# VCISwang/STCD

Hardware: AMD Instinct MI355X
Metric: image-pairs/sec (256x256 bf16 SiamUnet_diff train) (higher is better)
Workload: dtype bf16; 1 GPU; SiamUnet_diff(3,2) 256x256 full training step (fwd + cross_entropy + bwd + AdamW), 16 pairs/GPU, synthetic LEVIR-CD-shaped pairs resident in HBM; global_batch=16, image=256, parallelism=dp1

## Files before the change

### include/stcd_hip.h

```cpp
#ifndef STCD_HIP_H
#define STCD_HIP_H

#include <stdint.h>

#ifdef __cplusplus
extern "C" {
#endif

#define STCD_ABI_VERSION 2

#define STCD_ARCH_DIFF 0
#define STCD_ARCH_CONC 1
#define STCD_ARCH_SUB 2
#define STCD_ARCH_SNUNET 3
#define STCD_ARCH_SEGCD 4
#define STCD_ARCH_SEGCD_R18 5
#define STCD_ARCH_SEGCD_R34 6
#define STCD_ARCH_SEGCD_R101 7
#define STCD_ARCH_SEGCD_R152 8
#define STCD_ARCH_FCEF 9
#define STCD_ARCH_XCONC 10
#define STCD_ARCH_SNUNET_CONC 11
#define STCD_ARCH_SNUNET_CONC_DS 12
#define STCD_ARCH_UNETSEG 16
// ... 213 lines not shown
    int32_t bw_ldy;
    int32_t blocks, tiles_per_group, blocks_per_group, bn_rep;
    int32_t tile_m;
} stcd_conv_fused;
int stcd_op_conv_fused(const stcd_conv_geom* g, stcd_conv_fused* f, const void* in, const float* w, const float* bias, void* out,
                       void* scratch, int64_t scratch_bytes, void* hip_stream);
int stcd_op_wgrad(int dtype, int impl, const stcd_conv_geom* g, const void* in, const void* dout, float* dw,
                  void* scratch, int64_t scratch_bytes, void* hip_stream);
int64_t stcd_op_scratch_bytes(const stcd_conv_geom* g);

typedef struct stcd_map_geom {
    int32_t n, h, w, c, groups;
} stcd_map_geom;
int64_t stcd_op_ew_scratch_bytes(const stcd_map_geom* g);
int stcd_op_bn_act(int dtype, const stcd_map_geom* g, const void* y, int ldy, const float* gamma, const float* beta,
                   float* running_mean, float* running_var, const float* mask, int relu, int training, void* a, int lda,
                   void* pool, int ldp, float* stat, void* scratch, int64_t scratch_bytes, void* hip_stream);
int stcd_op_bn_act_pair(int dtype, const stcd_map_geom* g, const void* y, int ldy, const float* gamma, const float* beta,
                        float* running_mean, float* running_var, const float* mask, int fuse_mode, void* a, int lda, void* pool,
                        int ldp, void* fused, int ldf, float* stat, void* scratch, int64_t scratch_bytes, void* hip_stream);
int stcd_op_bn_act_bwd(int dtype, const stcd_map_geom* g, const void* da, int ldda, const void* y, int ldy, const float* stat,
                       const float* mask, int relu, void* dy, int lddy, float* dgamma, float* dbeta, void* scratch,
                       int64_t scratch_bytes, void* hip_stream);
int stcd_op_maxpool(int dtype, const stcd_map_geom* g, const void* a, int lda, void* pool, int ldp, void* hip_stream);
int stcd_op_maxpool_bwd(int dtype, const stcd_map_geom* g, const void* a, int lda, const void* dpool, int ldp, void* da, int ldda,
                        int accumulate, void* hip_stream);
int stcd_op_maxpool3(int dtype, const stcd_map_geom* g, const void* a, int lda, void* pool, int ldp, void* idx, void* hip_stream);
int stcd_op_maxpool3_bwd(int dtype, const stcd_map_geom* g, const void* idx, const void* dpool, int ldp, void* da, int ldda, void* hip_stream);
int64_t stcd_op_pairdw_scratch_bytes(const stcd_map_geom* g);
int stcd_op_pairdw(int dtype, const stcd_map_geom* g, const void* a, int lda, const float* w, const float* b, void* out, int ldo,
                   void* hip_stream);
int stcd_op_pairdw_bwd(int dtype, const stcd_map_geom* g, const void* a, int lda, const void* dout, int lddo, const float* w, void* da,
                       int ldda, float* dw, void* scratch, int64_t scratch_bytes, void* hip_stream);
int stcd_op_fuse(int dtype, int mode, const stcd_map_geom* g, const void* a, int lda, void* d, int ldd, void* hip_stream);
int stcd_op_fuse_bwd(int dtype, int mode, const stcd_map_geom* g, const void* a, int lda, const void* dd, int ldd, void* da, int ldda,
                     void* hip_stream);
int stcd_op_rep_pad(int dtype, const stcd_map_geom* g, void* d, int ld, int h0, int w0, void* hip_stream);
int stcd_op_rep_pad_bwd(int dtype, const stcd_map_geom* g, void* dd, int ld, int h0, int w0, void* hip_stream);
int stcd_op_skip_bwd(int dtype, int mode, const stcd_map_geom* g, const void* a, int lda, const void* y, int ldy, const void* dd,
                     int ldd, const void* dpool, int ldp, const float* stat, const float* mask, void* da, int ldda, void* dy,
                     int lddy, float* dgamma, float* dbeta, void* scratch, int64_t scratch_bytes, void* hip_stream);

int64_t stcd_op_cf_scratch_bytes(int64_t rows, int channels, int n, int q_tokens, int kv_tokens);
int stcd_op_cf_im2col(int dtype, const void* x, void* col, int ldc, int n, int h, int w, int c, int k, int stride, int pad, void* hip_stream);
int stcd_op_cf_col2im(int dtype, const void* dcol, int ldc, void* dx, int n, int h, int w, int c, int k, int stride, int pad, int accumulate,
                      void* hip_stream);
// ... 29 lines not shown
```

### stcd_amd/_lib.py

```python
from __future__ import annotations

import ctypes as C
import os

import torch

_HERE = os.path.dirname(os.path.abspath(__file__))
LIB_PATH = os.environ.get("STCD_LIB_PATH") or os.path.join(_HERE, "libstcd_hip.so")

ARCH_DIFF, ARCH_CONC, ARCH_SUB, ARCH_SNUNET, ARCH_SEGCD = 0, 1, 2, 3, 4
ARCH_SEGCD_R18, ARCH_SEGCD_R34, ARCH_SEGCD_R101, ARCH_SEGCD_R152 = 5, 6, 7, 8
ARCH_FCEF = 9
ARCH_XCONC = 10
ARCH_SNUNET_CONC = 11
ARCH_SNUNET_CONC_DS = 12
ARCH_UNETSEG = 16
ARCH_FFCTLCD = 32
ARCH_BASE_RESNET = 48
ARCH_BIT = 52
ARCH_CHANGEFORMER = 64
DTYPE_F32, DTYPE_BF16 = 0, 1
ARCH_IDS = {"diff": ARCH_DIFF, "conc": ARCH_CONC, "sub": ARCH_SUB, "fcef": ARCH_FCEF, "xconc": ARCH_XCONC, "snunet": ARCH_SNUNET, "snunet_conc": ARCH_SNUNET_CONC, "snunet_conc_ds": ARCH_SNUNET_CONC_DS, "segcd": ARCH_SEGCD,
            "segcd_resnet50": ARCH_SEGCD, "segcd_resnet18": ARCH_SEGCD_R18, "segcd_resnet34": ARCH_SEGCD_R34,
            "segcd_resnet101": ARCH_SEGCD_R101, "segcd_resnet152": ARCH_SEGCD_R152,
# ... 123 lines not shown
    "stcd_scene_gather_d4": (_i, [_vp, _vp, _i, _i, _i, _i, _i, _i, _i, C.POINTER(_f), C.POINTER(_f), _vp, _vp, _i, _vp]),
    "stcd_scene_stitch_d4": (_i, [_vp, _i, _i, _i, _i, _i, _i, _i, _i, _i, _vp, _vp, _vp, _i, _vp]),
    "stcd_scene_gather_one_d4": (_i, [_vp, _i, _i, _i, _i, _i, _i, _i, C.POINTER(_f), C.POINTER(_f), _vp, _i, _vp]),
    "stcd_scene_stitch_heads_d4": (_i, [C.POINTER(_vp), _i, _i, _i, _i, _i, _i, _i, _i, _i, _i, _vp, _vp, _vp, _i, _vp]),
    "stcd_scene_finalize_seg": (_i, [_vp, _vp, _i, _i, _i, _f, _f, _vp, _vp, _vp, _vp, _vp, _vp, _vp, _vp, _vp, _vp]),
    "stcd_selftrain_score": (_i, [C.POINTER(_vp), _i, _i, _i, _i64, _f, _vp, _i, _vp, _vp, _vp, _vp]),
    "stcd_scene_cell_agree": (_i, [C.POINTER(_vp), _i, _i, _i, _i, _i, _i, _vp, _vp, _vp, _vp]),
    "stcd_mask_close": (_i, [_vp, _i, _i, _i, _i, _vp, _vp]),
    "stcd_objects_scratch_bytes": (_i64, [_i, _i]),
    "stcd_objects_label": (_i, [_vp, _i, _i, _i, _i, _vp, _vp, _vp, _i64, _vp]),
    "stcd_objects_table": (_i, [_vp, _i, _i, _i, _vp, _vp, _vp, _vp, _vp]),
    "stcd_mask_filter_objects": (_i, [_vp, _i, _i, _i, _i64, _i64, _i, _vp, _vp, _i64, _vp]),
    "stcd_rings_scratch_bytes": (_i64, [_i, _i, _i64]),
    "stcd_rings_count": (_i, [_vp, _i, _i, _i, _i64, _vp, _vp, _i64, _vp]),
    "stcd_rings_write": (_i, [_vp, _i, _i, _i, _i64, _i64, _i64, _vp, _vp, _vp, _vp, _vp, _i64, _vp]),
    "stcd_op_conv": (_i, [_i, _i, C.POINTER(ConvGeom), _vp, _vp, _vp, _vp, _vp, _i64, _vp]),
    "stcd_op_conv_fused": (_i, [C.POINTER(ConvGeom), C.POINTER(ConvFused), _vp, _vp, _vp, _vp, _vp, _i64, _vp]),
    "stcd_op_wgrad": (_i, [_i, _i, C.POINTER(ConvGeom), _vp, _vp, _vp, _vp, _i64, _vp]),
    "stcd_op_scratch_bytes": (_i64, [C.POINTER(ConvGeom)]),
    "stcd_op_ew_scratch_bytes": (_i64, [C.POINTER(MapGeom)]),
    "stcd_op_bn_act": (_i, [_i, C.POINTER(MapGeom), _vp, _i, _vp, _vp, _vp, _vp, _vp, _i, _i, _vp, _i, _vp, _i, _vp, _vp, _i64, _vp]),
    "stcd_op_bn_act_pair": (_i, [_i, C.POINTER(MapGeom), _vp, _i, _vp, _vp, _vp, _vp, _vp, _i, _vp, _i, _vp, _i, _vp, _i, _vp, _vp, _i64, _vp]),
    "stcd_op_bn_act_bwd": (_i, [_i, C.POINTER(MapGeom), _vp, _i, _vp, _i, _vp, _vp, _i, _vp, _i, _vp, _vp, _vp, _i64, _vp]),
    "stcd_op_maxpool": (_i, [_i, C.POINTER(MapGeom), _vp, _i, _vp, _i, _vp]),
    "stcd_op_maxpool_bwd": (_i, [_i, C.POINTER(MapGeom), _vp, _i, _vp, _i, _vp, _i, _i, _vp]),
    "stcd_op_maxpool3": (_i, [_i, C.POINTER(MapGeom), _vp, _i, _vp, _i, _vp, _vp]),
    "stcd_op_maxpool3_bwd": (_i, [_i, C.POINTER(MapGeom), _vp, _vp, _i, _vp, _i, _vp]),
    "stcd_op_pairdw_scratch_bytes": (_i64, [C.POINTER(MapGeom)]),
    "stcd_op_pairdw": (_i, [_i, C.POINTER(MapGeom), _vp, _i, _vp, _vp, _vp, _i, _vp]),
    "stcd_op_pairdw_bwd": (_i, [_i, C.POINTER(MapGeom), _vp, _i, _vp, _i, _vp, _vp, _i, _vp, _vp, _i64, _vp]),
    "stcd_op_fuse": (_i, [_i, _i, C.POINTER(MapGeom), _vp, _i, _vp, _i, _vp]),
    "stcd_op_fuse_bwd": (_i, [_i, _i, C.POINTER(MapGeom), _vp, _i, _vp, _i, _vp, _i, _vp]),
    "stcd_op_rep_pad": (_i, [_i, C.POINTER(MapGeom), _vp, _i, _i, _i, _vp]),
    "stcd_op_rep_pad_bwd": (_i, [_i, C.POINTER(MapGeom), _vp, _i, _i, _i, _vp]),
    "stcd_op_skip_bwd": (_i, [_i, _i, C.POINTER(MapGeom), _vp, _i, _vp, _i, _vp, _i, _vp, _i, _vp, _vp, _vp, _i, _vp, _i, _vp, _vp, _vp, _i64, _vp]),
    "stcd_op_cf_scratch_bytes": (_i64, [_i64, _i, _i, _i, _i]),
    "stcd_op_cf_im2col": (_i, [_i, _vp, _vp, _i, _i, _i, _i, _i, _i, _i, _i, _vp]),
    "stcd_op_cf_col2im": (_i, [_i, _vp, _i, _vp, _i, _i, _i, _i, _i, _i, _i, _i, _vp]),
    "stcd_op_cf_layernorm": (_i, [_i, _vp, _vp, _vp, _vp, _vp, _i64, _i, _f, _vp]),
    "stcd_op_cf_layernorm_bwd": (_i, [_i, _vp, _vp, _vp, _vp, _vp, _vp, _vp, _vp, _vp, _vp, _i64, _i, _vp]),
    "stcd_op_cf_colsum": (_i, [_i, _vp, _i64, _i, _vp, _vp, _vp]),
    "stcd_op_cf_attention": (_i, [_i, _vp, _vp, _vp, _vp, _i, _i, _i, _i, _i, _f, C.c_uint64, _vp]),
    "stcd_op_cf_attention_scratch_bytes": (_i64, [_i, _i, _i, _i, _i]),
    "stcd_op_cf_attention_bwd": (_i, [_i, _vp, _vp, _vp, _vp, _vp, _vp, _vp, _vp, _i, _i, _i, _i, _i, _f, C.c_uint64, _vp]),
    "stcd_op_cf_dwgelu": (_i, [_i, _vp, _vp, _vp, _vp, _vp, _i, _i, _i, _i, _f, C.c_uint64, _vp]),
    "stcd_op_cf_dwgelu_scratch_bytes": (_i64, [_i, _i, _i, _i]),
# ... 36 lines not shown
```

### stcd_amd/csrc/common.h

```cpp
#pragma once
#include <hip/hip_runtime.h>
#include <stdint.h>
#include <stdio.h>
#include <stdlib.h>
#include <string>
#include <string.h>

#include "../../include/stcd_hip.h"

namespace stcd {

typedef __bf16 bf16;

enum DType { F32 = STCD_DTYPE_F32, BF16 = STCD_DTYPE_BF16 };
inline size_t dsize(int dt) { return dt == BF16 ? 2 : 4; }

void set_error(const std::string& msg);

static inline int env_int(const char* name, int dflt) { const char* v = getenv(name); return v ? atoi(v) : dflt; }
static inline bool env_flag(const char* name, bool dflt) { const char* v = getenv(name); return v && v[0] == (dflt ? '0' : '1') ? !dflt : dflt; }

#define STCD_CHECK_AS(fn, cond, msg)                                       \
    do {                                                                   \
        if (!(cond)) {                                                     \
// ... 277 lines not shown
                   float s1_scale = BN_FS1, float s2_scale = BN_FS2, const ConvEpi* epi = nullptr);
struct ConvHaloPlan {
    int NH = 0;
    int nslices = 0, P = 0, blocks = 0, lds_bytes = 0;
    bool ok = false;
};
ConvHaloPlan conv_halo_plan(const stcd_conv_geom& g, const ConvMfmaPlan& p);
int launch_conv_halo(const stcd_conv_geom& g, const ConvMfmaPlan& p, const ConvHaloPlan& hp, const void* in, const void* wf,
                     const float* bias, void* out, hipStream_t s, const ConvEpi* epi = nullptr);

struct ConvDmaPlan {
    int tiles_m = 0, tiles_n = 0, blocks = 0, lds_bytes = 0;
    bool ok = false;
};
ConvDmaPlan conv_dma_plan(const stcd_conv_geom& g, const ConvMfmaPlan& p);
int launch_conv_dma(const stcd_conv_geom& g, const ConvMfmaPlan& p, const ConvDmaPlan& dp, const void* in, const void* wf,
                    const float* bias, void* out, hipStream_t s, const ConvEpi* epi = nullptr);

bool conv_small_ok(const stcd_conv_geom& g, const ConvMfmaPlan& p);
int conv_small_blocks(const stcd_conv_geom& g, int groups);
int launch_conv_small(const stcd_conv_geom& g, const void* in, const void* wf_modeB, const float* bias, void* out,
                      bool out_nchw_f32, int groups, long long* stat_acc, int cpad, hipStream_t s, const XfSrc* xf = nullptr,
                      const BwdSum* bs = nullptr);
bool conv_small_call_ok(const stcd_conv_geom& g, int groups, const XfSrc* xf);
bool conv_small_bwdsum_ok(const stcd_conv_geom& g);
struct WgradMfmaPlan {
    int WCI = 1, NTW = 1, gx = 1, gy = 1, gz = 1;
    int64_t slab_floats = 0;
    int wi_valid = 0;
    int gemm = 0;
    int dma = 0;
    bool ok = false;
};
WgradMfmaPlan wgrad_mfma_plan(const stcd_conv_geom& g, int kpad, int wld, bool allow_wide = false, int force_co64 = -1);
int launch_wgrad_mfma(const stcd_conv_geom& g, const WgradMfmaPlan& p, const void* in, const void* dout, float* slab,
                      int kpad, int wld, hipStream_t s);
struct WgradJob {
    stcd_conv_geom g;
    int64_t in_off, dout_off, slab_off;
    int kpad, wld;
    int dymin, dxmin, HH, HWp;
    int tiles_x, tiles_y, ntiles;
    int xrow_bytes;
    int x_bytes, y_bytes;
    int co_valid;
    unsigned in_bytes, dout_bytes;
// ... 319 lines not shown
```

### stcd_amd/csrc/engine.hip

```cpp
#include <algorithm>
#include <climits>
#include <cstdint>
#include <array>
#include <cstring>
#include <memory>
#include <vector>

#include "common.h"

namespace stcd {

static thread_local std::string g_err;
void set_error(const std::string& msg) { g_err = msg; }

enum ConvKind { K_CONV3 = 0, K_CONVT3_S1 = 1, K_UPCONV = 2, K_CONV1 = 3, K_CONVT2 = 4, K_CONV3_S2 = 5, K_CONV1_S2 = 6, K_STEM7 = 7 };

struct TRef { int64_t off = -1; int ld = 0; };
struct GRef { int64_t off = -1; int ld = 0; int64_t goff = 0; };

static inline int round8(int c) { return (c + 7) & ~7; }

struct ConvW {
    std::string name;
    int kind = 0, cin = 0, cout = 0;
    int kin_p = 0, nout_p = 0;
    int64_t w_off = 0, b_off = 0;
    PackSpec fwd{}, dgrad{};
    int64_t wpk_fwd = -1, wpk_dgrad = -1, dwe = -1;
    int64_t dwe_floats = 0;
};
struct BnP {
    std::string name;
    int C = 0, calls = 1;
    int64_t g_off = 0, b_off = 0;
    int64_t run_off = 0;
};
struct DropP { std::string name; int rows = 0, C = 0; int64_t off = 0; };

struct ConvOp {
    stcd_conv_geom g{};
    int conv = -1; bool dgrad = false;
    int tap0 = 0;
    int kreal = 0, nreal = 0;
    ConvMfmaPlan plan; int64_t wf = -1;
    bool small = false;
    ConvResPlan res; int res_groups = 1;
    ConvGemmPlan gemm;
    ConvDmaPlan dma;
    ConvHaloPlan halo;
    ConvTilePlan tile;
};
struct WgradOp {
    stcd_conv_geom g{};
    int conv = -1, tap0 = 0, kreal = 0, nreal = 0;
    WgradMfmaPlan plan;
    int64_t slab = -1;
    int stage = 0;
    int64_t in_off = -1, dout_off = -1;
    bool grouped = false;
    int group = -1;
    int64_t xf_stat_off = -1, xf_mask_off = -1; int xf_C = 0, xf_groups = 1, xf_npg = 1;
    bool own_taps = false;
    int8_t oky[9] = {0}, okx[9] = {0};
};
struct WgradGroup {
    int WCI = 1, NTW = 1; bool t9 = false;
    bool xf = false;
    int gemm = 0;
// ... 945 lines not shown
                      (e.use_bwdsum && e.use_bwdsum_res) ? L.groups : 1);
    };
    for (auto& L : e.enc) bind_cbrd(L);
    for (auto& L : e.dec) bind_cbrd(L);
    for (auto& X : e.xc) bind_cbrd(X.res);
    for (auto& U : e.ups) {
        const ConvW& cv = e.convs[U.conv];
        for (int ph = 0; ph < 4; ++ph) {
            int tap0;
            const stcd_conv_geom g = geom_phase3(U.N, U.h, U.w, U.C, U.in.ld, U.Ho, U.Wo, U.C, U.out.ld, ph, cv.fwd, &tap0);
            bind.conv(U.fwd[ph], g, U.conv, false, tap0, U.C, U.C);
            bind.wgrad(U.wg[ph], g, U.conv, U.in.off, U.dOut.off, wg_stage(U.conv), tap0);
        }
        bind.conv(U.dgr, geom_gather2(U.N, U.Ho, U.Wo, cv.dgrad.kpad, U.dOut.ld, U.h, U.w, U.C, U.dIn.ld, cv.dgrad, 1), U.conv, true, 0, U.C, U.C);
    }
    {
        const ConvW& cv = e.convs[e.final_conv];
        bind.conv(e.final_fwd, geom3(B, H, W, cv.kin_p, e.finalIn.ld, e.label, e.label), e.final_conv, false, 0, cv.cin, e.label);
        bind.wgrad(e.final_wg, geom3(B, H, W, cv.kin_p, e.finalIn.ld, e.label, 8), e.final_conv, e.finalIn.off, e.G.off, wg_stage(e.final_conv));
        bind.conv(e.final_dgr, geom3(B, H, W, cv.dgrad.kpad, 8, cv.cin, e.dFinalIn.ld), e.final_conv, true, 0, e.label, cv.cin);
    }
    e.slab = ws.take(e.slab_floats * 4);

    for (auto& L : e.enc) { L.dgr_bwd = nullptr; L.bwd_sums_fused = false; }
    for (auto& L : e.dec) { L.dgr_bwd = nullptr; L.bwd_sums_fused = false; }
    e.final_dgr_bwd = nullptr;
    if (e.use_bwdsum && e.dt == BF16 && e.use_mfma && e.use_small && !e.use_virt) {
        const int res_too = e.use_bwdsum_res;
        auto dest_ok = [&](const Cbrd& P, const ConvOp& dgr, int64_t dIn_off, int dIn_ld, int N) {
            const bool kern = (dgr.small && conv_small_bwdsum_ok(dgr.g)) ||
                              (res_too && !dgr.small && !dgr.gemm.ok && e.use_res && dgr.res.ok && dgr.res_groups == P.groups &&
                               conv_res_bwdsum_ok(dgr.g, dgr.res));
            return !P.pool && P.fuse_dst.off < 0 && !P.virt && kern && dgr.wf >= 0 && dIn_off == P.dA.off && dIn_ld == P.dA.ld &&
                   e.convs[P.conv].cout == dgr.g.co && P.N == N && N % P.groups == 0 &&
                   (P.groups == 1 || P.dA.goff == (int64_t)P.npg * P.H * P.W * P.dA.ld);
        };
        auto scan = [&](std::vector<Cbrd>& v) {
            for (size_t i = 1; i < v.size(); ++i) {
                Cbrd& N = v[i]; Cbrd& P = v[i - 1];
                if (N.has_dIn && N.dgr_sum_acc < 0 && dest_ok(P, N.dgr, N.dIn.off, N.dIn.ld, N.N)) { N.dgr_bwd = &P; P.bwd_sums_fused = true; }
            }
        };
        scan(e.enc); scan(e.dec);
        if (!e.dec.empty() && dest_ok(e.dec.back(), e.final_dgr, e.dFinalIn.off, e.dFinalIn.ld, e.dec.back().N)) {
            e.final_dgr_bwd = &e.dec.back(); e.dec.back().bwd_sums_fused = true;
        }
// ... 132 lines not shown

static bool mfma_on(const stcd_engine& e) { return e.dt == BF16 && e.use_mfma; }

struct StatReq { long long* acc = nullptr; int groups = 1; int c0 = 0; int C = 0; float s1 = BN_FS1, s2 = BN_FS2; };

enum class ConvKernel { REF, MFMA, SMALL, RES, TILE, GEMM, HALO, DMA };
constexpr unsigned conv_kernel_bit(ConvKernel k) { return 1u << (int)k; }
struct ConvCall {
    bool nchw = false;
    int stat_groups = 0;
    bool bn_form = false;
    const XfSrc* xf = nullptr;
    bool bwd = false;
    unsigned allowed = ~0u;
};
static int conv_small_groups(const ConvCall& k) {
    return (k.xf && k.xf->on) ? k.xf->groups : (k.stat_groups > 0 && k.bn_form) ? k.stat_groups : 1;
}
static ConvKernel conv_kernel(bool mfma, bool use_small, const ConvOp& op, const ConvCall& k) {
    auto may = [&](ConvKernel x) { return (k.allowed & conv_kernel_bit(x)) != 0; };
    if (conv_on_ref(mfma, op)) return ConvKernel::REF;
    const bool xf_on = k.xf && k.xf->on, stats = k.stat_groups > 0;
    const bool small = op.small && use_small;
    if (k.bwd) return small ? ConvKernel::SMALL : ConvKernel::RES;
    if (op.gemm.ok && !k.nchw) {
        if (op.dma.ok && op.res_groups == 1 && !stats && may(ConvKernel::DMA)) return ConvKernel::DMA;
        if (op.halo.ok && !stats && may(ConvKernel::HALO)) return ConvKernel::HALO;
        return ConvKernel::GEMM;
    }
    if (small && conv_small_call_ok(op.g, conv_small_groups(k), k.xf)) return ConvKernel::SMALL;
    if (op.res.ok && !k.nchw && !small) {
        if (op.tile.ok && !xf_on && may(ConvKernel::TILE)) return ConvKernel::TILE;
        if (!xf_on || conv_res_xf_ok(op.g, op.res, op.res_groups, *k.xf)) return ConvKernel::RES;
    }
    return ConvKernel::MFMA;
}
static void conv_kernel_name(ConvKernel kern, const ConvOp& op, bool bwd, char (&kname)[64]) {
    switch (kern) {
        case ConvKernel::DMA: snprintf(kname, sizeof(kname), "k_conv_dma"); break;
        case ConvKernel::HALO: snprintf(kname, sizeof(kname), "k_conv_halo"); break;
        case ConvKernel::GEMM: snprintf(kname, sizeof(kname), "k_conv_gemm<%d>", op.gemm.W); break;
        case ConvKernel::TILE: snprintf(kname, sizeof(kname), "k_conv_tile<%d>", op.tile.NT); break;
        case ConvKernel::RES:
            if (bwd) snprintf(kname, sizeof(kname), "k_conv_res<bwd>");
            else snprintf(kname, sizeof(kname), "k_conv_res<%d, %d, %s>", op.res.NT, op.res.CW, op.res.single_halo ? "true" : "false");
            break;
        case ConvKernel::SMALL:
            if (bwd) snprintf(kname, sizeof(kname), "k_conv_small<bwd>");
            else snprintf(kname, sizeof(kname), "k_conv_small<1, %d>", (op.g.ntaps * op.g.ci + 31) / 32 <= 5 ? 5 : 9);
            break;
        case ConvKernel::MFMA: snprintf(kname, sizeof(kname), "k_conv_mfma<%d>", op.plan.NT); break;
        case ConvKernel::REF: snprintf(kname, sizeof(kname), "k_conv_ref"); break;
    }
}

static void exec_conv(const Ctx& c, const ConvOp& op, const void* in, const float* bias, void* out, bool nchw,
                      const StatReq* sr = nullptr, int* stat_chunks = nullptr, const ConvEpi* epi = nullptr, int* epi_fused = nullptr,
                      const XfSrc* xf = nullptr, const BwdSum* bs = nullptr) {
    const ConvW& cv = c.e.convs[op.conv];
    long long* stat_acc = sr ? sr->acc : nullptr;
    ConvCall call;
    call.nchw = nchw; call.xf = xf; call.bwd = bs != nullptr;
    call.stat_groups = stat_acc ? sr->groups : 0;
    call.bn_form = sr && sr->c0 == 0 && sr->C == op.g.co && sr->s1 == BN_FS1 && sr->s2 == BN_FS2;
    const ConvKernel kern = conv_kernel(mfma_on(c.e), c.e.use_small, op, call);
    double fl, by;
    conv_work(c.e, op.g, op.kreal, op.nreal, &fl, &by);
    if (bs) by += (double)op.g.n * op.g.ho * op.g.wo * op.g.co * 2.0;
    char kname[64];
    conv_kernel_name(kern, op, bs != nullptr, kname);
    ProfScope prof(c, PC_CONV, fl, by, kname);
// ... 307 lines not shown
        StatReq sr;
        if (L.dgr_sum_acc >= 0) { sr.acc = c.at<long long>(L.dgr_sum_acc); sr.groups = 1; sr.c0 = L.dgr_sum_c0; sr.C = L.dgr_sum_C; sr.s1 = sr.s2 = BN_BS; }
        BwdSum bs;
        if (L.dgr_bwd) bs = bwd_sum_of(c, *L.dgr_bwd);
        exec_conv(c, L.dgr, c.at(L.dY.off), nullptr, c.at(L.dIn.off), false, L.dgr_sum_acc >= 0 ? &sr : nullptr, nullptr, nullptr, nullptr, nullptr,
                  L.dgr_bwd ? &bs : nullptr);
    }
}

static void upconv_forward(const Ctx& c, const UpConv& U) {
    stcd_engine& e = c.e;
    const ConvW& cv = e.convs[U.conv];
    if (!exec_conv_x4(c, U.fwd, c.at(U.in.off), c.params + cv.b_off, c.at(U.out.off)))
        for (int ph = 0; ph < 4; ++ph) exec_conv(c, U.fwd[ph], c.at(U.in.off), c.params + cv.b_off, c.at(U.out.off), false);
    launch_rep_pad(e.dt, c.at(U.out.off), U.out.ld, U.N, U.Ho, U.Wo, 2 * U.h, 2 * U.w, U.C, c.s);
}

static void upconv_backward(const Ctx& c, const UpConv& U) {
    stcd_engine& e = c.e;
    const ConvW& cv = e.convs[U.conv];
    launch_rep_pad_bwd(e.dt, c.at(U.dOut.off), U.dOut.ld, U.N, U.Ho, U.Wo, 2 * U.h, 2 * U.w, U.C, c.s);
    if (U.bias_fused && mfma_on(e)) {
    } else if (2 * U.h == U.Ho && 2 * U.w == U.Wo) {
        launch_bias_grad(e.dt, c.at(U.dOut.off), U.dOut.ld, (int64_t)U.N * U.Ho * U.Wo, U.C, c.grads + cv.b_off, c.s,
                         e.dt == BF16 ? c.at<long long>(U.bias_acc) : nullptr);
    } else {
        const int64_t T = (int64_t)dsize(e.dt);
        for (int n = 0; n < U.N; ++n)
            for (int y = 0; y < 2 * U.h; ++y)
                launch_bias_grad(e.dt, c.at<char>(U.dOut.off) + ((int64_t)(n * U.Ho + y) * U.Wo) * U.dOut.ld * T, U.dOut.ld,
                                 2 * U.w, U.C, c.grads + cv.b_off, c.s, e.dt == BF16 ? c.at<long long>(U.bias_acc) : nullptr);
    }
    for (int ph = 0; ph < 4; ++ph) exec_wgrad(c, U.wg[ph], c.at(U.in.off), c.at(U.dOut.off));
    exec_conv(c, U.dgr, c.at(U.dOut.off), nullptr, c.at(U.dIn.off), false);
}

static void xconc_forward(const Ctx& c, const XConc& X, const Cbrd& skip, float* bn_running, bool training) {
    stcd_engine& e = c.e;
    const BnP& bn = e.bns[X.bn1];
    const int C = X.C, B = X.res.N, h = X.res.H, w = X.res.W;
    {
        ProfScope ps(c, PC_POOL_FUSE, 0.0, 3.0 * B * h * w * C * (double)dsize(e.dt), "k_pairdw_fwd");
        launch_pairdw_fwd(e.dt, c.at(skip.A.off), skip.A.ld, skip.A.goff, c.at(X.G.off), X.G.ld, c.params + X.w_off, c.params + X.b_off, B, h, w, C, c.s);
    }
    if (training) launch_bn_stats(e.dt, c.at(X.G.off), X.G.ld, C, 1, (int64_t)B * h * w, c.at<long long>(X.facc1), c.s);
    BnActArgs a;
    a.Y = c.at(X.G.off); a.ldy = X.G.ld;
// ... 1943 lines not shown
    if (epi_on) {
        STCD_CHECK(!f->gate || (f->ldg >= g->co && f->ldg % 8 == 0), "gate: the pixel stride must be a multiple of 8 and >= co");
        STCD_CHECK(!f->res || (f->ldr >= g->co && f->ldr % 8 == 0), "res: the pixel stride must be a multiple of 8 and >= co");
        STCD_CHECK(f->res || (f->alpha == 1.f && f->beta == 1.f), "alpha / beta combine the output with a residual: without one they must be 1");
        epi.relu = f->relu ? 1 : 0;
        epi.gate = f->gate; epi.ldg = f->ldg; epi.res = f->res; epi.ldr = f->ldr; epi.alpha = f->alpha; epi.beta = f->beta;
    }
    BwdSum bs;
    if (bwd) {
        STCD_CHECK(f->bw_y && f->bw_stat, "BatchNorm-backward sums need the layer's conv output and its statistics");
        STCD_CHECK(f->bw_ldy >= g->co && f->bw_ldy % 4 == 0, "bw_y: the pixel stride must be a multiple of 4 and >= co");
        bs.Y = f->bw_y; bs.ldy = f->bw_ldy; bs.stat = f->bw_stat; bs.mask = f->bw_mask; bs.acc = (long long*)f->bw_acc; bs.groups = groups;
    }
    const ConvMfmaPlan p = conv_mfma_plan(*g);
    STCD_CHECK(p.ok, "geometry not supported by the MFMA kernels");
    STCD_CHECK(scratch && scratch_bytes >= p.wf_elems * 2, "scratch too small for the fragment-order filter");
    hipStream_t s = (hipStream_t)hip_stream;
    long long* const acc = (long long*)f->sum_acc;
    const int sC = sums ? f->sum_c : g->co, sc0 = sums ? f->sum_c0 : 0;
    const float s1 = sums ? f->sum_scale1 : BN_FS1, s2 = sums ? f->sum_scale2 : BN_FS2;
    const int64_t tiles16 = (int64_t)g->n * ((g->hm + 15) / 16) * ((g->wm + 15) / 16);
    ConvResPlan rp; ConvTilePlan tp; ConvGemmPlan gp; ConvHaloPlan hp; ConvDmaPlan dp;
    if (k_small) {
        STCD_CHECK(conv_small_ok(*g, p) && conv_small_call_ok(*g, groups, nullptr), "geometry not supported by k_conv_small (one n-tile, <= 5 k-steps)");
        STCD_CHECK(!bwd || conv_small_bwdsum_ok(*g), "k_conv_small forms BatchNorm-backward sums for 16 channels out, whole 8 x 16 tiles, 3 or 5 k-steps");
        f->blocks = conv_small_blocks(*g, groups);
        f->blocks_per_group = f->blocks / groups;
        f->tiles_per_group = (int)((int64_t)g->n * ((g->hm + 7) / 8) * ((g->wm + 15) / 16) / groups);
    } else if (k_res) {
        rp = conv_res_plan(*g, p, groups);
        STCD_CHECK(rp.ok, "geometry not supported by k_conv_res (3x3 stride 1, Ci % 32 == 0)");
        STCD_CHECK(!bwd || conv_res_bwdsum_ok(*g, rp), "this k_conv_res plan forms no BatchNorm-backward sums (slices of one or two n-tiles, double halo)");
        f->blocks = rp.blocks; f->blocks_per_group = rp.P; f->tiles_per_group = (int)(tiles16 / groups);
    } else if (k_tile) {
        tp = conv_tile_plan(*g, p, groups);
        STCD_CHECK(tp.ok, "geometry not supported by k_conv_tile (3x3 stride 1 over the full map, Ci % 64 == 0, Co % 16 == 0)");
        f->blocks = tp.blocks; f->blocks_per_group = tp.P; f->tiles_per_group = (int)(tiles16 / groups);
    } else if (k_gemm) {
        gp = conv_gemm_plan(*g, p, groups);
        STCD_CHECK(gp.ok, "geometry not supported by k_conv_gemm (Ci % 64 == 0, Co % 64 == 0)");
        f->blocks = gp.blocks; f->blocks_per_group = gp.tiles_m; f->tiles_per_group = gp.tiles_m; f->tile_m = 32 * gp.W;
    } else if (k_halo) {
        hp = conv_halo_plan(*g, p);
        STCD_CHECK(hp.ok, "geometry not supported by k_conv_halo (3x3 stride 1, Ci % 128 == 0, Co % 128 == 0)");
        f->blocks = hp.blocks; f->blocks_per_group = hp.P; f->tiles_per_group = (int)tiles16;
    } else {
        dp = conv_dma_plan(*g, p);
// ... 67 lines not shown
```

### stcd_amd/csrc/kernels_conv_mfma.hip

```cpp
#include "common.h"

namespace stcd {

typedef __attribute__((ext_vector_type(8))) __bf16 bf16x8;
typedef __attribute__((ext_vector_type(4))) float f32x4;
typedef __attribute__((ext_vector_type(4))) unsigned u32x4;

struct ConvMfmaArgs {
    stcd_conv_geom g;
    const bf16* in;
    const bf16* wf;
    const float* bias;
    void* out;
    int out_nchw;
    int CiB, nchunks, KS;
    int modeB;
    int NTtot;
    int dymin, dxmin, HH, HWp, swmask;
    int tiles_x, tiles_y;
    int halo_bytes, wbuf_bytes;
    int tap[9];
};

static inline void fill_taps(const stcd_conv_geom& g, int* tap) {
// ... 1224 lines not shown
        __syncthreads();
        for (int i = tid; i < NT * 16 * 2; i += 256) {
            const int which = i / (NT * 16), c = i - which * NT * 16;
            const int t2 = c >> 4, qq = (c >> 2) & 3, j = c & 3;
            float acc_ = 0.f;
#pragma unroll
            for (int w = 0; w < 4; ++w) acc_ += red[(((w * NT + t2) * 4 + qq) * 4 + j) * 2 + which];
            if (c < a.cpad) bn_acc_add(a.stat_acc, bl, a.groups, a.cpad, grp, which, c, acc_, which ? a.s2_scale : a.s1_scale);
        }
    }
}

bool conv_small_ok(const stcd_conv_geom& g, const ConvMfmaPlan& p) {
    if (!p.ok || (!p.modeB && p.nchunks != 1)) return false;
    const int K = g.ntaps * g.ci;
    const int ks = (K + 31) / 32;
    const int nt = (g.co + 15) / 16;
    int dymin, dymax, dxmin, dxmax;
    taps_extent(g, &dymin, &dymax, &dxmin, &dxmax);
    const int HH = 7 * g.in_stride + (dymax - dymin) + 1, HWp = 15 * g.in_stride + (dxmax - dxmin) + 1;
    return ks <= 5 && nt <= 1 && g.ci <= 32 && HH * HWp * (g.ci / 8) <= 3 * 256;
}

int conv_small_blocks(const stcd_conv_geom& g, int groups) {
    const int64_t ntiles = (int64_t)g.n * ((g.hm + 7) / 8) * ((g.wm + 15) / 16);
    int64_t per_group = ntiles / groups;
    int64_t bpg = std::min<int64_t>(per_group, 2048 / groups);
    if (bpg < 1) bpg = 1;
    return (int)(bpg * groups);
}

bool conv_small_bwdsum_ok(const stcd_conv_geom& g) {
    const int ks = (g.ntaps * g.ci + 31) / 32;
    return g.co == 16 && g.hm % 8 == 0 && g.wm % 16 == 0 && g.hm == g.ho && g.wm == g.wo && g.out_stride == 1 && g.oy0 == 0 && g.ox0 == 0 &&
           (ks == 3 || ks == 5);
}
bool conv_small_call_ok(const stcd_conv_geom& g, int groups, const XfSrc* xf) {
    if (groups < 1 || g.n % groups != 0) return false;
    return !(xf && xf->on) || (xf->C == g.ci && xf->groups == groups);
}
int launch_conv_small(const stcd_conv_geom& g, const void* in, const void* wf_modeB, const float* bias, void* out,
                      bool out_nchw, int groups, long long* stat_acc, int cpad, hipStream_t s, const XfSrc* xf, const BwdSum* bs) {
    ConvSmallArgs a;
    a.bw_Y = nullptr; a.bw_ldy = 0; a.bw_stat = nullptr; a.bw_mask = nullptr; a.s1_scale = BN_FS1; a.s2_scale = BN_FS2;
    a.g = g;
    a.in = (const bf16*)in; a.wf = (const bf16*)wf_modeB; a.bias = bias; a.out = out; a.out_nchw = out_nchw ? 1 : 0;
// ... 1 lines not shown
    a.KS = (g.ntaps * g.ci + 31) / 32;
    const int nt = (g.co + 15) / 16;
    a.NTtot = nt;
    int dymax, dxmax;
    taps_extent(g, &a.dymin, &dymax, &a.dxmin, &dxmax);
    a.HH = 7 * g.in_stride + (dymax - a.dymin) + 1;
    a.HWp = 15 * g.in_stride + (dxmax - a.dxmin) + 1;
    a.tiles_x = (g.wm + 15) / 16;
    a.tiles_y = (g.hm + 7) / 8;
    a.ntiles = g.n * a.tiles_x * a.tiles_y;
    a.groups = groups;
    a.halo_bytes = (a.HH * a.HWp * g.ci * 2 + 255) & ~255;
    a.stat_acc = stat_acc;
    a.cpad = cpad;
    fill_taps(g, a.tap);
    if (!conv_small_call_ok(g, groups, xf)) return 1;
    const int blocks = conv_small_blocks(g, groups);
    size_t lds = std::max<size_t>(2 * (size_t)a.halo_bytes, 4 * 2 * 16 * 2 * 4 * 2);
    const bool use_xf = xf && xf->on;
    if (use_xf) {
        a.xf = *xf;
        lds = 2 * (size_t)a.halo_bytes + (size_t)xf->groups * 2 * xf->C * 4;
    }
    if (bs) {
        if (!conv_small_bwdsum_ok(g) || out_nchw || use_xf || nt != 1 || stat_acc || bs->groups != groups || !bs->acc) return 1;
        a.bw_Y = (const bf16*)bs->Y; a.bw_ldy = bs->ldy; a.bw_stat = bs->stat; a.bw_mask = bs->mask;
        a.stat_acc = bs->acc; a.cpad = g.co; a.s1_scale = BN_BS; a.s2_scale = BN_BS;
        if (a.KS == 3) k_conv_small<1, 3, false, 2, true><<<blocks, 256, lds, s>>>(a);
        else k_conv_small<1, 5, false, 2, true><<<blocks, 256, lds, s>>>(a);
        return 0;
    }
    if (nt != 1) return 1;
    const bool full = !out_nchw && g.co == nt * 16 && g.hm % 8 == 0 && g.wm % 16 == 0;
#define LAUNCH_SMALL(N_, K_, F_) do { if (use_xf) k_conv_small<N_, K_, true, F_><<<blocks, 256, lds, s>>>(a); else k_conv_small<N_, K_, false, F_><<<blocks, 256, lds, s>>>(a); } while (0)
#define LAUNCH_SMALL_K(N_, K_) do { if (full) LAUNCH_SMALL(N_, K_, 2); else LAUNCH_SMALL(N_, K_, 1); } while (0)
#define LAUNCH_SMALL_N(N_) do { \
        if (a.KS == 3) LAUNCH_SMALL_K(N_, 3); \
        else if (a.KS == 5) LAUNCH_SMALL_K(N_, 5); \
        else if (a.KS <= 5) LAUNCH_SMALL(N_, 5, 0); \
        else if (a.KS == 9) LAUNCH_SMALL_K(N_, 9); \
        else LAUNCH_SMALL(N_, 9, 0); } while (0)
    LAUNCH_SMALL_N(1);
#undef LAUNCH_SMALL_K
#undef LAUNCH_SMALL_N
#undef LAUNCH_SMALL
    return 0;
}

struct ConvResArgs {
    stcd_conv_geom g;
    const bf16* in;
    const bf16* wf;
    const float* bias;
    bf16* out;
    int NTtot, KSp;
// ... 993 lines not shown
```

### stcd_amd/csrc/ops_abi.hip

```cpp
#include <algorithm>

#include "common.h"

using namespace stcd;

namespace {

int check_map(const stcd_map_geom* g) {
    STCD_CHECK(g != nullptr, "geometry is null");
    STCD_CHECK(g->n >= 1 && g->h >= 1 && g->w >= 1, "bad sizes");
    STCD_CHECK(g->c >= 8 && g->c % 8 == 0 && g->c <= 2048 && (g->c & (g->c - 1)) == 0, "channels must be a power of two in [8, 2048]");
    STCD_CHECK(g->groups >= 1 && g->groups <= 2 && g->n % g->groups == 0, "groups must be 1 or 2 and divide n");
    STCD_CHECK((int64_t)g->n * g->h * g->w * (g->c / 8) < ((int64_t)1 << 31), "tensor too large for 32-bit indexing");
    return 0;
}

int64_t acc_bytes(const stcd_map_geom& g) { return bn_acc_bytes(g.groups, g.c); }

}

extern "C" {

int64_t stcd_op_ew_scratch_bytes(const stcd_map_geom* g) {
    if (!g || g->c < 8 || g->groups < 1) return 0;
// ... 48 lines not shown
    aa.Y = y; aa.ldy = ldy; aa.A = a; aa.lda = lda; aa.a_group_off = ppg * lda;
    aa.P = pool; aa.ldp = ldp; aa.stat = stat; aa.mask = mask;
    aa.C = g->c; aa.groups = 2; aa.npg = npg; aa.H = g->h; aa.W = g->w; aa.relu = 1;
    launch_bn_act_pair(dtype, aa, fused, ldf, fuse_mode, s);
    STCD_HIP(hipGetLastError());
    return 0;
}

int stcd_op_bn_act_bwd(int dtype, const stcd_map_geom* g, const void* da, int ldda, const void* y, int ldy, const float* stat,
                       const float* mask, int relu, void* dy, int lddy, float* dgamma, float* dbeta, void* scratch,
                       int64_t scratch_bytes, void* hip_stream) {
    if (check_map(g)) return 1;
    STCD_CHECK(dtype == STCD_DTYPE_F32 || dtype == STCD_DTYPE_BF16, "unknown dtype");
    STCD_CHECK(da && y && stat && dy && dgamma && dbeta && scratch, "null pointer argument");
    STCD_CHECK(scratch_bytes >= stcd_op_ew_scratch_bytes(g), "scratch too small");
    hipStream_t s = (hipStream_t)hip_stream;
    const int npg = g->n / g->groups;
    const int64_t HW = (int64_t)g->h * g->w, ppg = npg * HW;
    long long* acc = (long long*)scratch;
    STCD_HIP(hipMemsetAsync(acc, 0, (size_t)acc_bytes(*g), s));
    launch_bn_bwd_reduce(dtype, da, ldda, ppg * ldda, y, ldy, stat, mask, g->c, g->groups, npg, HW, relu ? 1 : 0, acc, s);
    launch_bn_bwd_apply(dtype, da, ldda, ppg * ldda, dy, lddy, y, ldy, stat, acc, dgamma, dbeta, mask, g->c, g->groups, npg, HW,
                        relu ? 1 : 0, s);
    STCD_HIP(hipGetLastError());
    return 0;
}

int stcd_op_maxpool(int dtype, const stcd_map_geom* g, const void* a, int lda, void* pool, int ldp, void* hip_stream) {
    if (check_map(g)) return 1;
    STCD_CHECK(a && pool, "null pointer argument");
    launch_maxpool(dtype, a, lda, pool, ldp, g->n, g->h, g->w, g->c, (hipStream_t)hip_stream);
    STCD_HIP(hipGetLastError());
    return 0;
}

int stcd_op_maxpool_bwd(int dtype, const stcd_map_geom* g, const void* a, int lda, const void* dpool, int ldp, void* da, int ldda,
                        int accumulate, void* hip_stream) {
    if (check_map(g)) return 1;
    STCD_CHECK(a && dpool && da, "null pointer argument");
    const int npg = g->n / g->groups;
    const int64_t ppg = (int64_t)npg * g->h * g->w;
    launch_pool_bwd(dtype, a, lda, ppg * lda, dpool, ldp, da, ldda, ppg * ldda, g->groups, npg, g->h, g->w, g->c, accumulate ? 1 : 0,
                    (hipStream_t)hip_stream);
    STCD_HIP(hipGetLastError());
    return 0;
}
// ... 216 lines not shown
```

Before: 8031 image-pairs/sec.

## Route wide 16->32 dgrad convs to small kernel and offload bias grad

Adds a 'wide' path that sends large 3x3 stride-1 16->32-channel data-gradient convolutions through k_conv_small with two n-tiles, in place of the residual/MFMA kernels. Separately, in the upsample backward the bias-gradient reduction is forked onto the side weight-gradient stream so it can overlap with main-stream work. Also exposes a channel_sums ABI entry for statistics and bias sums, which looks like a test hook. The risks are that the small kernel may be slower for these shapes and that the extra event record and wait add sync overhead.

After: 8086 image-pairs/sec, median of 6. Within noise of the previous version (+0.7%).

```diff
diff --git a/include/stcd_hip.h b/include/stcd_hip.h
--- a/include/stcd_hip.h
+++ b/include/stcd_hip.h
@@ -259,6 +259,8 @@
 int stcd_op_bn_act_bwd(int dtype, const stcd_map_geom* g, const void* da, int ldda, const void* y, int ldy, const float* stat,
                        const float* mask, int relu, void* dy, int lddy, float* dgamma, float* dbeta, void* scratch,
                        int64_t scratch_bytes, void* hip_stream);
+int stcd_op_channel_sums(int kind, const stcd_map_geom* g, const void* x, int ldx, const void* y, int ldy, const float* stat,
+                         const float* mask, void* acc, void* hip_stream);
 int stcd_op_maxpool(int dtype, const stcd_map_geom* g, const void* a, int lda, void* pool, int ldp, void* hip_stream);
 int stcd_op_maxpool_bwd(int dtype, const stcd_map_geom* g, const void* a, int lda, const void* dpool, int ldp, void* da, int ldda,
                         int accumulate, void* hip_stream);
diff --git a/stcd_amd/_lib.py b/stcd_amd/_lib.py
--- a/stcd_amd/_lib.py
+++ b/stcd_amd/_lib.py
@@ -169,6 +169,7 @@
     "stcd_op_bn_act": (_i, [_i, C.POINTER(MapGeom), _vp, _i, _vp, _vp, _vp, _vp, _vp, _i, _i, _vp, _i, _vp, _i, _vp, _vp, _i64, _vp]),
     "stcd_op_bn_act_pair": (_i, [_i, C.POINTER(MapGeom), _vp, _i, _vp, _vp, _vp, _vp, _vp, _i, _vp, _i, _vp, _i, _vp, _i, _vp, _vp, _i64, _vp]),
     "stcd_op_bn_act_bwd": (_i, [_i, C.POINTER(MapGeom), _vp, _i, _vp, _i, _vp, _vp, _i, _vp, _i, _vp, _vp, _vp, _i64, _vp]),
+    "stcd_op_channel_sums": (_i, [_i, C.POINTER(MapGeom), _vp, _i, _vp, _i, _vp, _vp, _vp, _vp]),
     "stcd_op_maxpool": (_i, [_i, C.POINTER(MapGeom), _vp, _i, _vp, _i, _vp]),
     "stcd_op_maxpool_bwd": (_i, [_i, C.POINTER(MapGeom), _vp, _i, _vp, _i, _vp, _i, _i, _vp]),
     "stcd_op_maxpool3": (_i, [_i, C.POINTER(MapGeom), _vp, _i, _vp, _i, _vp, _vp]),
diff --git a/stcd_amd/csrc/common.h b/stcd_amd/csrc/common.h
--- a/stcd_amd/csrc/common.h
+++ b/stcd_amd/csrc/common.h
@@ -323,6 +323,8 @@
 int launch_conv_small(const stcd_conv_geom& g, const void* in, const void* wf_modeB, const float* bias, void* out,
                       bool out_nchw_f32, int groups, long long* stat_acc, int cpad, hipStream_t s, const XfSrc* xf = nullptr,
                       const BwdSum* bs = nullptr);
+constexpr int64_t CONV_SMALL_WIDE_MIN = 1048576;
+bool conv_small_wide_ok(const stcd_conv_geom& g);
 bool conv_small_call_ok(const stcd_conv_geom& g, int groups, const XfSrc* xf);
 bool conv_small_bwdsum_ok(const stcd_conv_geom& g);
 struct WgradMfmaPlan {
diff --git a/stcd_amd/csrc/engine.hip b/stcd_amd/csrc/engine.hip
--- a/stcd_amd/csrc/engine.hip
+++ b/stcd_amd/csrc/engine.hip
@@ -44,6 +44,7 @@
     int kreal = 0, nreal = 0;
     ConvMfmaPlan plan; int64_t wf = -1;
     bool small = false;
+    bool wide = false;
     ConvResPlan res; int res_groups = 1;
     ConvGemmPlan gemm;
     ConvDmaPlan dma;
@@ -1035,6 +1036,17 @@
     }
     e.slab = ws.take(e.slab_floats * 4);
 
+    if (e.dt == BF16 && e.use_mfma && e.use_small && !(e.debug_flags & 4)) {
+        auto bind_wide = [&](Cbrd& L) {
+            const ConvOp& op = L.dgr;
+            L.dgr.wide = L.has_dIn && !op.small && op.plan.ok && op.wf >= 0 && conv_small_wide_ok(op.g) &&
+                         (int64_t)op.g.n * op.g.hm * op.g.wm >= CONV_SMALL_WIDE_MIN;
+        };
+        for (auto& L : e.enc) bind_wide(L);
+        for (auto& L : e.dec) bind_wide(L);
+        for (auto& X : e.xc) bind_wide(X.res);
+    }
+
     for (auto& L : e.enc) { L.dgr_bwd = nullptr; L.bwd_sums_fused = false; }
     for (auto& L : e.dec) { L.dgr_bwd = nullptr; L.bwd_sums_fused = false; }
     e.final_dgr_bwd = nullptr;
@@ -1213,13 +1225,14 @@
     if (conv_on_ref(mfma, op)) return ConvKernel::REF;
     const bool xf_on = k.xf && k.xf->on, stats = k.stat_groups > 0;
     const bool small = op.small && use_small;
+    const bool wide = op.wide && use_small && !xf_on && !k.nchw && !stats;
     if (k.bwd) return small ? ConvKernel::SMALL : ConvKernel::RES;
     if (op.gemm.ok && !k.nchw) {
         if (op.dma.ok && op.res_groups == 1 && !stats && may(ConvKernel::DMA)) return ConvKernel::DMA;
         if (op.halo.ok && !stats && may(ConvKernel::HALO)) return ConvKernel::HALO;
         return ConvKernel::GEMM;
     }
-    if (small && conv_small_call_ok(op.g, conv_small_groups(k), k.xf)) return ConvKernel::SMALL;
+    if ((small || wide) && conv_small_call_ok(op.g, conv_small_groups(k), k.xf)) return ConvKernel::SMALL;
     if (op.res.ok && !k.nchw && !small) {
         if (op.tile.ok && !xf_on && may(ConvKernel::TILE)) return ConvKernel::TILE;
         if (!xf_on || conv_res_xf_ok(op.g, op.res, op.res_groups, *k.xf)) return ConvKernel::RES;
@@ -1237,7 +1250,8 @@
             else snprintf(kname, sizeof(kname), "k_conv_res<%d, %d, %s>", op.res.NT, op.res.CW, op.res.single_halo ? "true" : "false");
             break;
         case ConvKernel::SMALL:
-            if (bwd) snprintf(kname, sizeof(kname), "k_conv_small<bwd>");
+            if (op.wide) snprintf(kname, sizeof(kname), "k_conv_small<2, 5>");
+            else if (bwd) snprintf(kname, sizeof(kname), "k_conv_small<bwd>");
             else snprintf(kname, sizeof(kname), "k_conv_small<1, %d>", (op.g.ntaps * op.g.ci + 31) / 32 <= 5 ? 5 : 9);
             break;
         case ConvKernel::MFMA: snprintf(kname, sizeof(kname), "k_conv_mfma<%d>", op.plan.NT); break;
@@ -1591,7 +1605,12 @@
     launch_rep_pad_bwd(e.dt, c.at(U.dOut.off), U.dOut.ld, U.N, U.Ho, U.Wo, 2 * U.h, 2 * U.w, U.C, c.s);
     if (U.bias_fused && mfma_on(e)) {
     } else if (2 * U.h == U.Ho && 2 * U.w == U.Wo) {
-        launch_bias_grad(e.dt, c.at(U.dOut.off), U.dOut.ld, (int64_t)U.N * U.Ho * U.Wo, U.C, c.grads + cv.b_off, c.s,
+        hipStream_t bs = c.s;
+        if (e.wg_cur_side && e.dt == BF16 && !(e.debug_flags & 8)) {
+            if (hipEventRecord(e.wg_fork, c.s) != hipSuccess || hipStreamWaitEvent(e.wg_cur_side, e.wg_fork, 0) != hipSuccess) { set_error("side-stream fork failed"); return; }
+            bs = e.wg_cur_side;
+        }
+        launch_bias_grad(e.dt, c.at(U.dOut.off), U.dOut.ld, (int64_t)U.N * U.Ho * U.Wo, U.C, c.grads + cv.b_off, bs,
                          e.dt == BF16 ? c.at<long long>(U.bias_acc) : nullptr);
     } else {
         const int64_t T = (int64_t)dsize(e.dt);
@@ -3581,7 +3600,8 @@
     const int64_t tiles16 = (int64_t)g->n * ((g->hm + 15) / 16) * ((g->wm + 15) / 16);
     ConvResPlan rp; ConvTilePlan tp; ConvGemmPlan gp; ConvHaloPlan hp; ConvDmaPlan dp;
     if (k_small) {
-        STCD_CHECK(conv_small_ok(*g, p) && conv_small_call_ok(*g, groups, nullptr), "geometry not supported by k_conv_small (one n-tile, <= 5 k-steps)");
+        STCD_CHECK((conv_small_ok(*g, p) || conv_small_wide_ok(*g)) && conv_small_call_ok(*g, groups, nullptr),
+                   "geometry not supported by k_conv_small (one n-tile, <= 5 k-steps; or whole tiles, 9 taps, stride 1, 16 -> 32 channels)");
         STCD_CHECK(!bwd || conv_small_bwdsum_ok(*g), "k_conv_small forms BatchNorm-backward sums for 16 channels out, whole 8 x 16 tiles, 3 or 5 k-steps");
         f->blocks = conv_small_blocks(*g, groups);
         f->blocks_per_group = f->blocks / groups;
diff --git a/stcd_amd/csrc/kernels_conv_mfma.hip b/stcd_amd/csrc/kernels_conv_mfma.hip
--- a/stcd_amd/csrc/kernels_conv_mfma.hip
+++ b/stcd_amd/csrc/kernels_conv_mfma.hip
@@ -1270,6 +1270,15 @@
     return ks <= 5 && nt <= 1 && g.ci <= 32 && HH * HWp * (g.ci / 8) <= 3 * 256;
 }
 
+bool conv_small_wide_ok(const stcd_conv_geom& g) {
+    if (g.ci != 16 || g.co != 32 || g.ntaps != 9 || g.in_stride != 1 || g.ldi % 8 != 0 || g.ldo % 4 != 0) return false;
+    if (g.hm % 8 != 0 || g.wm % 16 != 0) return false;
+    if (g.out_stride != 1 || g.oy0 != 0 || g.ox0 != 0 || g.ho != g.hm || g.wo != g.wm) return false;
+    int dymin, dymax, dxmin, dxmax;
+    taps_extent(g, &dymin, &dymax, &dxmin, &dxmax);
+    return (7 + (dymax - dymin) + 1) * (15 + (dxmax - dxmin) + 1) * 2 <= 3 * 256;
+}
+
 int conv_small_blocks(const stcd_conv_geom& g, int groups) {
     const int64_t ntiles = (int64_t)g.n * ((g.hm + 7) / 8) * ((g.wm + 15) / 16);
     int64_t per_group = ntiles / groups;
@@ -1317,6 +1326,8 @@
         a.xf = *xf;
         lds = 2 * (size_t)a.halo_bytes + (size_t)xf->groups * 2 * xf->C * 4;
     }
+    const bool wide = nt != 1 && conv_small_wide_ok(g);
+    if (nt != 1 && (!wide || out_nchw || use_xf || bs)) return 1;
     if (bs) {
         if (!conv_small_bwdsum_ok(g) || out_nchw || use_xf || nt != 1 || stat_acc || bs->groups != groups || !bs->acc) return 1;
         a.bw_Y = (const bf16*)bs->Y; a.bw_ldy = bs->ldy; a.bw_stat = bs->stat; a.bw_mask = bs->mask;
@@ -1325,7 +1336,10 @@
         else k_conv_small<1, 5, false, 2, true><<<blocks, 256, lds, s>>>(a);
         return 0;
     }
-    if (nt != 1) return 1;
+    if (wide) {
+        k_conv_small<2, 5, false, 2><<<blocks, 256, lds, s>>>(a);
+        return 0;
+    }
     const bool full = !out_nchw && g.co == nt * 16 && g.hm % 8 == 0 && g.wm % 16 == 0;
 #define LAUNCH_SMALL(N_, K_, F_) do { if (use_xf) k_conv_small<N_, K_, true, F_><<<blocks, 256, lds, s>>>(a); else k_conv_small<N_, K_, false, F_><<<blocks, 256, lds, s>>>(a); } while (0)
 #define LAUNCH_SMALL_K(N_, K_) do { if (full) LAUNCH_SMALL(N_, K_, 2); else LAUNCH_SMALL(N_, K_, 1); } while (0)
diff --git a/stcd_amd/csrc/ops_abi.hip b/stcd_amd/csrc/ops_abi.hip
--- a/stcd_amd/csrc/ops_abi.hip
+++ b/stcd_amd/csrc/ops_abi.hip
@@ -94,6 +94,28 @@
     launch_bn_bwd_reduce(dtype, da, ldda, ppg * ldda, y, ldy, stat, mask, g->c, g->groups, npg, HW, relu ? 1 : 0, acc, s);
     launch_bn_bwd_apply(dtype, da, ldda, ppg * ldda, dy, lddy, y, ldy, stat, acc, dgamma, dbeta, mask, g->c, g->groups, npg, HW,
                         relu ? 1 : 0, s);
+    STCD_HIP(hipGetLastError());
+    return 0;
+}
+
+int stcd_op_channel_sums(int kind, const stcd_map_geom* g, const void* x, int ldx, const void* y, int ldy, const float* stat,
+                         const float* mask, void* acc, void* hip_stream) {
+    if (check_map(g)) return 1;
+    STCD_CHECK(kind >= 0 && kind <= 2, "kind must be 0 (statistics), 1 (BatchNorm-backward sums) or 2 (bias gradient)");
+    STCD_CHECK(x && acc, "null pointer argument");
+    STCD_CHECK(ldx >= g->c && ldx % 8 == 0, "bad pixel stride");
+    hipStream_t s = (hipStream_t)hip_stream;
+    const int npg = g->n / g->groups;
+    const int64_t HW = (int64_t)g->h * g->w, ppg = npg * HW;
+    if (kind == 0) {
+        launch_bn_stats(STCD_DTYPE_BF16, x, ldx, g->c, g->groups, ppg, (long long*)acc, s);
+    } else if (kind == 1) {
+        STCD_CHECK(y && stat && ldy >= g->c && ldy % 8 == 0, "BatchNorm-backward sums need the layer's conv output and its statistics");
+        launch_bn_bwd_reduce(STCD_DTYPE_BF16, x, ldx, ppg * ldx, y, ldy, stat, mask, g->c, g->groups, npg, HW, 1, (long long*)acc, s);
+    } else {
+        STCD_CHECK(g->groups == 1, "the bias gradient sums one group");
+        launch_bias_grad(STCD_DTYPE_BF16, x, ldx, (int64_t)g->n * HW, g->c, nullptr, s, (long long*)acc);
+    }
     STCD_HIP(hipGetLastError());
     return 0;
 }
```
